# rgalljamov/DRLoco

Hardware: NVIDIA B200
Metric: env-steps/s incl. DeepMimic reward (higher is better)
Workload: dtype f32

## Files before the change

drloco_b200/csrc/fd_tree.cuh:

```cuda
#pragma once
#include "fd_common.cuh"

namespace drl {

template <int NV>
struct Topo;

template <>
struct Topo<14> {
  static constexpr int NB = 7, NCHAIN = 2, KMAX = 4, NROOT = 6, NSLIDE = 3;
  __host__ __device__ static constexpr int nd(int k) { return k == 0 ? 6 : (k == 1 ? 2 : 1); }
  __host__ __device__ static constexpr int dof_off(int k) { return k <= 1 ? 0 : (k == 2 ? 2 : (k == 3 ? 3 : 4)); }
  __host__ __device__ static constexpr int chain_dof0(int c) { return c == 0 ? 6 : 10; }
  __host__ __device__ static constexpr int chain_body1(int c) { return c == 0 ? 1 : 4; }
  __host__ __device__ static constexpr int chain_len(int) { return 4; }
  __host__ __device__ static constexpr int axis(int k, int s) { return k == 0 ? s : (k == 1 ? (s == 0 ? 1 : 0) : 1); }
  __host__ __device__ static constexpr int chain_of(int j) { return (j - 6) / 4; }
  static constexpr int NBOX = 2;
  __host__ __device__ static constexpr int box_body(int bx) { return bx == 0 ? 3 : 6; }
};

template <>
struct Topo<19> {
  static constexpr int NB = 8, NCHAIN = 3, KMAX = 4, NROOT = 6, NSLIDE = 3;
  __host__ __device__ static constexpr int nd(int k) { return k == 0 ? 6 : (k == 1 ? 3 : 1); }
  __host__ __device__ static constexpr int dof_off(int k) { return k <= 1 ? 0 : (k == 2 ? 3 : (k == 3 ? 4 : 5)); }
  __host__ __device__ static constexpr int chain_dof0(int c) { return c == 0 ? 9 : (c == 1 ? 14 : 6); }
  __host__ __device__ static constexpr int chain_body1(int c) { return c == 0 ? 2 : (c == 1 ? 5 : 1); }
  __host__ __device__ static constexpr int chain_len(int c) { return c == 2 ? 2 : 4; }
  __host__ __device__ static constexpr int axis(int k, int s) { return k == 0 ? s : (k == 1 ? (s == 2 ? 2 : -1) : 1); }
  __host__ __device__ static constexpr int chain_of(int j) { return j < 9 ? 2 : (j < 14 ? 0 : 1); }
  static constexpr int NBOX = 4;
  __host__ __device__ static constexpr int box_body(int bx) { return bx == 0 ? 0 : (bx == 1 ? 1 : (bx == 2 ? 4 : 7)); }
};

template <int NV>
__host__ __device__ constexpr unsigned body_subtree_mask(int b) {
  using T = Topo<NV>;
  if (b == 0) return (1u << T::NB) - 1u;
  unsigned m = 0;
  for (int c = 0; c < T::NCHAIN; c++)
    for (int k = 1; k < T::chain_len(c); k++) {
      const int x = T::chain_body1(c) + k - 1;
      if (x == b)
        for (int k2 = k; k2 < T::chain_len(c); k2++) m |= 1u << (T::chain_body1(c) + k2 - 1);
    }
  return m;
}

template <int NV>
__host__ __device__ constexpr bool dof_is_anc(int r, int k) {
  return r < k && (r < Topo<NV>::NROOT || Topo<NV>::chain_of(r) == Topo<NV>::chain_of(k));
}
template <int NV>
__host__ __device__ constexpr unsigned dof_anc_mask(int k) {
  unsigned m = 0;
  for (int r = 0; r < k; r++)
    if (dof_is_anc<NV>(r, k)) m |= 1u << r;
  return m;
}

template <int NV>
__host__ __device__ constexpr unsigned dof_desc_mask(int k) {
  unsigned m = 0;
  for (int c = k + 1; c < NV; c++)
    if (dof_is_anc<NV>(k, c)) m |= 1u << c;
  return m;
}

template <int NV, int G>
__device__ __forceinline__ float ldl_solve_tree(float (&H)[NV + 1], int l) {
  float invd = 0.f;
  const unsigned me = 1u << l;
#pragma unroll
  for (int k = NV - 1; k >= 0; k--) {
    const float dk = __shfl_sync(kFull, H[k], k, G);
    const float inv = fast_rcp(fmaxf(dk, 1e-30f));
    const float lck = H[k] * inv;
    const bool upd = (dof_anc_mask<NV>(k) & me) != 0u;
    if (l == k) invd = inv;
#pragma unroll
    for (int r = 0; r <= NV; r++) {
      if (r == NV || dof_is_anc<NV>(r, k)) {
        const float vr = __shfl_sync(kFull, H[r], k, G);
        if (upd) H[r] = fmaf(-vr, lck, H[r]);
      }
    }
  }
  float sacc = H[NV], x = 0.f;
#pragma unroll
  for (int k = 0; k < NV; k++) {
    const float xk = __shfl_sync(kFull, sacc * invd, k, G);
    if (dof_desc_mask<NV>(k) & me) sacc = fmaf(-H[k], xk, sacc);
    if (l == k) x = xk;
  }
  return x;
}

constexpr int kWredBox = 29;

template <int G>
struct EnvSmem {
  static constexpr int kWredHalf = (G == 16 ? 2 * kWredBox * 4 + 8 : 4 * kWredBox * 4);
  static_assert(kWredHalf % 32 == 16, "bank layout of the staging buffer");
  float v[G];
  float acc[G];
  float tau[G];
  float cssn[G][2];
  float S[G][12];
  union {
    struct {
      float Fd[G][12];
      float bodyR[kMaxBody][16];
      float Ib[kMaxBody][12];
      float axw[G][4];
    };
    struct {
      float Wred[2 * kWredHalf];
      float sph[G][12];
    };
  };
  float Ic[kMaxBody][12];
  union {
    struct {
      float V[kMaxBody][8];
      float Ab[kMaxBody][8];
      float T[kMaxBody][8];
      float W[kMaxBody][24];
      float U[kMaxBody][8];
    };
    float Mt[kMaxBody * 56];
  };
  float obsbuf[kMaxObs];
  int cnt[4];
  float pad_[(G == 16) ? 20 : 4];
};
static_assert((sizeof(EnvSmem<16>) / 4) % 32 == 8, "environment stride must be 8 mod 32 floats (bank layout)");
static_assert(sizeof(EnvSmem<16>) % 16 == 0 && sizeof(EnvSmem<32>) % 16 == 0, "vector loads need 16-byte rows");

struct ChainLane {
  int c3, row;
  int c6, comp;
};

__device__ __forceinline__ void rot_row(int ax, float& R0, float& R1, float& R2, float c, float s) {
  if (ax == 0) { const float u = R1, w = R2; R1 = c * u + s * w; R2 = c * w - s * u; }
  else if (ax == 1) { const float u = R2, w = R0; R2 = c * u + s * w; R0 = c * w - s * u; }
  else { const float u = R0, w = R1; R0 = c * u + s * w; R1 = c * w - s * u; }
}

template <int NV, int G>
__device__ __forceinline__ void tree_kinematics(const DevModel& M, EnvSmem<G>& E, const ChainLane& C, int l) {
  using T = Topo<NV>;
  if (l < 3 * T::NCHAIN) {
    const int c = C.c3, r = C.row;
    const int cd0 = T::chain_dof0(c), cb1 = T::chain_body1(c), clen = T::chain_len(c);
    float R0 = r == 0 ? 1.f : 0.f, R1 = r == 1 ? 1.f : 0.f, R2 = r == 2 ? 1.f : 0.f, pr = 0.f;
#pragma unroll
    for (int k = 0; k < T::KMAX; k++) {
      if (k < clen) {
        const int b = k == 0 ? 0 : cb1 + k - 1;
        const bool own = k > 0 || c == 0;
        if (k > 0) pr = pr + R0 * M.body_pos[b][0] + R1 * M.body_pos[b][1] + R2 * M.body_pos[b][2];
        const int j0 = k == 0 ? T::NSLIDE : cd0 + T::dof_off(k);
#pragma unroll
        for (int s = 0; s < 3; s++) {
          if (s < (k == 0 ? T::NROOT - T::NSLIDE : T::nd(k))) {
            const int j = j0 + s;
            const int code = M.dof_code[j];
            const float2 cs = *reinterpret_cast<const float2*>(&E.cssn[j][0]);
            const int a = T::axis(k, s) >= 0 ? T::axis(k, s) : (code & 3);
            const float ax = a == 0 ? R0 : (a == 1 ? R1 : R2);
            if (own) E.axw[j][r] = (code & 4) ? -ax : ax;
            rot_row(a, R0, R1, R2, cs.x, cs.y);
          }
        }
        if (own) *reinterpret_cast<float4*>(&E.bodyR[b][4 * r]) = make_float4(R0, R1, R2, pr);
      }
    }
  }
  __syncwarp();
}

template <int G>
__device__ __forceinline__ float body_point_z(const EnvSmem<G>& E, int b, const float* p) {
  const float4 r2 = *reinterpret_cast<const float4*>(&E.bodyR[b][8]);
  return r2.w + r2.x * p[0] + r2.y * p[1] + r2.z * p[2];
}

template <int NV, int G, bool PRE>
__device__ __forceinline__ void chain_prefix(EnvSmem<G>& E, const float* coef, float (*dst)[8], int c, int comp,
                                             float init) {
  using T = Topo<NV>;
  const int cd0 = T::chain_dof0(c), cb1 = T::chain_body1(c), clen = T::chain_len(c);
  float acc = init;
#pragma unroll
  for (int k = 0; k < T::KMAX; k++) {
    if (k < clen) {
      const int b = k == 0 ? 0 : cb1 + k - 1;
      const int j0 = k == 0 ? 0 : cd0 + T::dof_off(k);
      const bool own = k > 0 || c == 0;
#pragma unroll
      for (int s = 0; s < 6; s++) {
        if (s < T::nd(k)) {
          const int j = j0 + s;
          if (PRE && own) E.Fd[j][comp] = acc;
          acc = fmaf(coef[j], E.S[j][comp], acc);
        }
      }
      if (own) dst[b][comp] = acc;
    }
  }
}

template <int NV, int G>
__device__ __forceinline__ void chain_prefix_rows(EnvSmem<G>& E, float (*dst)[8], int c, int comp, float init) {
  using T = Topo<NV>;
  const int cd0 = T::chain_dof0(c), cb1 = T::chain_body1(c), clen = T::chain_len(c);
  float acc = init;
#pragma unroll
  for (int k = 0; k < T::KMAX; k++) {
    if (k < clen) {
      const int b = k == 0 ? 0 : cb1 + k - 1;
      const int j0 = k == 0 ? 0 : cd0 + T::dof_off(k);
#pragma unroll
      for (int s = 0; s < 6; s++)
        if (s < T::nd(k)) acc += E.Fd[j0 + s][comp];
      if (k > 0 || c == 0) dst[b][comp] = acc;
    }
  }
}

template <int NV>
__device__ __forceinline__ void subtree_scan(const float* src, float* dst, int stride, unsigned present) {
  using T = Topo<NV>;
  float root = (present & 1u) ? src[0] : 0.f;
#pragma unroll
  for (int c = 0; c < T::NCHAIN; c++) {
    float s = 0.f;
#pragma unroll
    for (int k = T::KMAX - 1; k >= 1; k--) {
      if (k < T::chain_len(c)) {
        const int b = T::chain_body1(c) + k - 1;
        if ((present >> b) & 1u) s += src[b * stride];
        dst[b * stride] = s;
      }
    }
    root += s;
  }
  dst[0] = root;
}

struct Contact {
  float Px, Py, Pz, D, mu, ar[4];
};
__device__ __forceinline__ void st_contact(float* p, const Contact& c) {
  *reinterpret_cast<float4*>(p) = make_float4(c.Px, c.Py, c.Pz, c.D);
  *reinterpret_cast<float4*>(p + 4) = make_float4(c.mu, c.ar[0], c.ar[1], c.ar[2]);
  p[8] = c.ar[3];
}
__device__ __forceinline__ Contact ld_contact(const float* p) {
  const float4 a = *reinterpret_cast<const float4*>(p), b = *reinterpret_cast<const float4*>(p + 4);
  return Contact{a.x, a.y, a.z, a.w, b.x, {b.y, b.z, b.w, p[8]}};
}

template <int G, bool BOX>
__device__ __forceinline__ void contact_setup(const DevModel& M, const EnvSmem<G>& E, int s, int b, float dist,
                                              Contact& c) {
  const float4 r0 = *reinterpret_cast<const float4*>(&E.bodyR[b][0]);
  const float4 r1 = *reinterpret_cast<const float4*>(&E.bodyR[b][4]);
  const float4 r2 = *reinterpret_cast<const float4*>(&E.bodyR[b][8]);
  const float x = M.cand_pos[s][0], y = M.cand_pos[s][1], z = M.cand_pos[s][2];
  if (BOX) {
    const float ux = M.cand_aux[s][0], uy = M.cand_aux[s][1], uz = M.cand_aux[s][2];
    c.Px = (r0.w + r0.x * ux + r0.y * uy + r0.z * uz) + (r0.x * x + r0.y * y + r0.z * z);
    c.Py = (r1.w + r1.x * ux + r1.y * uy + r1.z * uz) + (r1.x * x + r1.y * y + r1.z * z);
    c.Pz = (r2.w + r2.x * ux + r2.y * uy + r2.z * uz) + (r2.x * x + r2.y * y + r2.z * z) - 0.5f * dist;
  } else {
    const float rad = M.cand_aux[s][0];
    c.Px = r0.w + (r0.x * x + r0.y * y + r0.z * z);
    c.Py = r1.w + (r1.x * x + r1.y * y + r1.z * z);
    c.Pz = r2.w + (r2.x * x + r2.y * y + r2.z * z) - rad - 0.5f * dist;
  }
  const float mu = M.cand_mu[s];
  const float imp = impedance(M, dist);
  const float Rn = fmaxf(kMinVal, (1.f - imp) * M.body_invw_tran[b] * (1.f + mu * mu));
  c.D = imp * fast_rcp(2.f * mu * mu * Rn);
  c.mu = mu;
  const Vec6 Vb = ld6(E.V[b]);
  float ux, uy, uz;
  cross3(ux, uy, uz, Vb.w0, Vb.w1, Vb.w2, c.Px, c.Py, c.Pz);
// ... 204 lines not shown
  __syncwarp();
  float rhs0 = 0.f;
  if (L.isdof) {
    const float cb = dot6(S, ld6(E.Ab[L.body]));
    rhs0 = tau - M.dof_damping[l] * v - cb;
    if (DBG) { dbg[0 * 32 + l] = cb; dbg[1 * 32 + l] = rhs0; }
  }
  float lsg = 0.f, lD = 0.f, laref = 0.f;
  if (L.isdof && M.dof_limited[l]) {
    float dist = 0.f;
    const float lo = M.dof_lo[l], hi = M.dof_hi[l];
    if (q < lo) { lsg = 1.f; dist = q - lo; }
    else if (q > hi) { lsg = -1.f; dist = hi - q; }
    if (lsg != 0.f) {
      const float imp = impedance(M, dist);
      lD = imp * fast_rcp(fmaxf(kMinVal, (1.f - imp) * M.dof_invw[l]));
      laref = -M.Bc * lsg * v - M.Kc * imp * dist;
    }
  }
  if (!act0) AS.bits[0] = 0u;
  else if (!(AS.prev_act & 1u)) AS.bits[0] = 0xFu;
  if (!act1) AS.bits[1] = 0u;
  else if (!(AS.prev_act & 2u)) AS.bits[1] = 0xFu;
  if (lsg == 0.f) AS.lbit = false;
  else if (!AS.prev_lim) AS.lbit = true;
  const bool any_limit = __any_sync(kFull, lsg != 0.f);
  const bool constrained = (conmask != 0u) || any_limit;
  unsigned subcon = 0u;
#pragma unroll
  for (int b = 0; b < T::NB; b++)
    if (body_subtree_mask<NV>(b) & conmask) subcon |= 1u << b;
  int n_iter = 0;
  bool capped = false;
  if (solver_barrier) __syncthreads();
  float H[NV + 1];
  for (int it = 0; it < kMaxSolverIter; it++) {
    if (constrained) n_iter++;
    if (conmask != 0u) {
      float wv[28];
      contact_hessian(c0, act0 ? AS.bits[0] : 0u, wv);
      if (l < M.nbox_cand) {
        float* dst = &E.Wred[((l >> 2) & 1) * ES::kWredHalf + (l >> 3) * kWredBox * 4 + (l & 3)];
#pragma unroll
        for (int i = 0; i < 27; i++) dst[i * 4] = wv[i];
      }
      __syncwarp();
      if (!sph_any) {
#pragma unroll
        for (int i0 = 0; i0 < 27; i0 += G) {
          const int i = i0 + l;
          if (i < 27) {
            float sb[T::NBOX];
#pragma unroll
            for (int bx = 0; bx < T::NBOX; bx++) {
              const float4 x0 = *reinterpret_cast<const float4*>(&E.Wred[(bx * kWredBox + i) * 4]);
              const float4 x1 = *reinterpret_cast<const float4*>(&E.Wred[ES::kWredHalf + (bx * kWredBox + i) * 4]);
              sb[bx] = ((x0.x + x0.y) + (x0.z + x0.w)) + ((x1.x + x1.y) + (x1.z + x1.w));
            }
#pragma unroll
            for (int b = 0; b < T::NB; b++) {
              float tot = 0.f;
              bool any = false;
#pragma unroll
              for (int bx = 0; bx < T::NBOX; bx++)
                if ((body_subtree_mask<NV>(b) >> T::box_body(bx)) & 1u) { tot = any ? tot + sb[bx] : sb[bx]; any = true; }
              if (any) {
                if (i < 21) E.W[b][i] = tot; else E.U[b][i - 21] = tot;
              }
            }
          }
        }
        __syncwarp();
      } else {
        for (unsigned mk = conmask & ~M.box_body_mask; mk; mk &= mk - 1) {
          const int b = __ffs(mk) - 1;
          for (int i = l; i < 24; i += G) E.W[b][i] = 0.f;
          if (l < 8) E.U[b][l] = 0.f;
        }
#pragma unroll
        for (int bx = 0; bx < T::NBOX; bx++) {
#pragma unroll
          for (int i0 = 0; i0 < 27; i0 += G) {
            const int i = i0 + l;
            if (i < 27) {
              const float4 x0 = *reinterpret_cast<const float4*>(&E.Wred[(bx * kWredBox + i) * 4]);
              const float4 x1 = *reinterpret_cast<const float4*>(&E.Wred[ES::kWredHalf + (bx * kWredBox + i) * 4]);
              const float sum = ((x0.x + x0.y) + (x0.z + x0.w)) + ((x1.x + x1.y) + (x1.z + x1.w));
              const int b = T::box_body(bx);
              if (i < 21) E.W[b][i] = sum; else E.U[b][i - 21] = sum;
            }
          }
        }
        {
          float wv1[28];
          Contact c1 = {0.f, 0.f, 0.f, 0.f, 0.f, {0.f, 0.f, 0.f, 0.f}};
          const unsigned bt = act1 ? AS.bits[1] : 0u;
          if (bt) c1 = ld_contact(E.sph[l]);
          contact_hessian(c1, bt, wv1);
          const int b1 = M.cand_body[G + l < M.ncand ? G + l : 0];
          __syncwarp();
          for (unsigned sm = __ballot_sync(kFull, bt != 0u); sm; sm &= sm - 1) {
            if (wl == __ffs(sm) - 1) {
              float* Wb = E.W[b1];
              float* Ub = E.U[b1];
#pragma unroll
              for (int i = 0; i < 21; i++) Wb[i] += wv1[i];
#pragma unroll
              for (int i = 0; i < 6; i++) Ub[i] += wv1[21 + i];
            }
            __syncwarp();
          }
        }
        __syncwarp();
        const unsigned present = conmask | M.box_body_mask;
        for (int i = l; i < 27; i += G) {
          if (i < 21) subtree_scan<NV>(&E.W[0][i], &E.W[0][i], 24, present);
          else subtree_scan<NV>(&E.U[0][i - 21], &E.U[0][i - 21], 8, present);
        }
        __syncwarp();
      }
    }
    H[NV] = rhs0;
    if (L.isdof) {
      Vec6 F = inertia_mul(E.Ic[L.body], S);
      if ((subcon >> L.body) & 1u) {
        float Wl[24];
#pragma unroll
        for (int i = 0; i < 24; i += 4) {
          const float4 t = *reinterpret_cast<const float4*>(&E.W[L.body][i]);
          Wl[i] = t.x; Wl[i + 1] = t.y; Wl[i + 2] = t.z; Wl[i + 3] = t.w;
        }
        const float Sv[6] = {S.w0, S.w1, S.w2, S.v0, S.v1, S.v2};
        float y[6];
#pragma unroll
        for (int i = 0; i < 6; i++) {
          float t = 0.f;
#pragma unroll
          for (int j = 0; j < 6; j++) t = fmaf(Wl[sym6(i, j)], Sv[j], t);
          y[i] = t;
        }
        F.w0 += y[0]; F.w1 += y[1]; F.w2 += y[2]; F.v0 += y[3]; F.v1 += y[4]; F.v2 += y[5];
        H[NV] += dot6(S, ld6(E.U[L.body]));
      }
      st6(E.Fd[l], F);
    }
    __syncwarp();
    mass_column<NV, G>(M, E, L, S, H);
    if (AS.lbit) {
#pragma unroll
      for (int r = 0; r < NV; r++)
        if (r == l) H[r] += lD;
      H[NV] += lD * lsg * laref;
    }
    a = ldl_solve_tree<NV, G>(H, l);
    if (!L.isdof) a = 0.f;
    if (L.isdof) E.acc[l] = a;
    if (!constrained) break;
    __syncwarp();
    if (conmask != 0u) {
      if (iscomp) chain_prefix<NV, G, false>(E, E.acc, E.T, C.c6, C.comp, 0.f);
      __syncwarp();
    }
    bool changed = false;
    if (act0) {
      const unsigned nb = contact_rows(c0, ld6(E.T[body0]));
      changed = nb != AS.bits[0];
      AS.bits[0] = nb;
    }
    if (sph_any) {
      if (act1) {
        const Contact c1 = ld_contact(E.sph[l]);
        const unsigned nb = contact_rows(c1, ld6(E.T[M.cand_body[G + l]]));
        changed = changed || (nb != AS.bits[1]);
        AS.bits[1] = nb;
      }
    }
    {
      const bool nl = (lsg != 0.f) && (lsg * a - laref < 0.f);
      changed = changed || (nl != AS.lbit);
      AS.lbit = nl;
    }
    if (!__any_sync(kFull, changed)) break;
    if (it == kMaxSolverIter - 1 && env_any(changed, L.emask)) capped = true;
    __syncwarp();
  }
  AS.prev_act = (act0 ? 1u : 0u) | (act1 ? 2u : 0u);
  AS.prev_lim = lsg != 0.f;
  if (l == 0) { E.cnt[0] += n_iter; E.cnt[1] += capped ? 1 : 0; }
  if (DBG) {
    dbg[(2 + NV) * 32 + l] = a;
    if (l == 0) {
      dbg[(3 + NV) * 32 + 0] = zO;
      dbg[(3 + NV) * 32 + 1] = (float)__popc(conmask);
    }
    dbg[(4 + NV) * 32 + l] = (float)((act0 ? 1 : 0) + (act1 ? 1 : 0));
  }
}

template <int NV, int G>
__device__ __forceinline__ void pure_mass_column(const DevModel& M, EnvSmem<G>& E, const LaneConst& L,
                                                  const Vec6& S, float (&H)[NV + 1]) {
  __syncwarp();
  if (L.isdof) st6(E.Fd[L.l], inertia_mul(E.Ic[L.body], S));
  __syncwarp();
  mass_column<NV, G>(M, E, L, S, H);
  __syncwarp();
}

}
```

drloco_b200/csrc/mimic_step.cu:

```cuda
#include "fd_common.cuh"
#include "fd_tree.cuh"

namespace drl {

__device__ __forceinline__ unsigned long long mix64(unsigned long long x) {
  x += 0x9E3779B97F4A7C15ull;
  x = (x ^ (x >> 30)) * 0xBF58476D1CE4E5B9ull;
  x = (x ^ (x >> 27)) * 0x94D049BB133111EBull;
  return x ^ (x >> 31);
}

struct Cursor {
  int i_step, pos, count, ep_dur, rsi_step, n_det, resets, flags;
};

constexpr int kFlagReadStep0 = 4, kFlagDetEpisode = 8;
__device__ __forceinline__ int data_step(const Cursor& c) { return (c.flags & kFlagReadStep0) ? 0 : c.i_step; }
__device__ __forceinline__ int shift_step(const Cursor& c) { return (c.flags & kFlagDetEpisode) ? 0 : c.rsi_step; }

__device__ __forceinline__ void cursor_next(const DevModel& M, const StepArgs& A, Cursor& c, float& dist) {
  const int len = A.step_len[data_step(c)];
  c.pos += M.increment;
  if (M.cursor_mode == DRL_CURSOR_STEPWISE) {
    const int dif = c.pos - len + 1;
// ... 264 lines not shown
  float zO = M.root_z0;
  for (int j = 0; j < M.nslide; j++) zO = fmaf(M.dof_slide_z[j], E.cssn[j][1], zO);
  tree_kinematics<NV, G>(M, E, CL, l);
  float sz = 3.0e38f;
  for (int s = l; s < M.nsite; s += G) sz = fminf(sz, zO + body_point_z<G>(E, M.site_body[s], M.site_pos[s]));
  const float lowest = group_min<G>(sz);
  if (l == M.com_z_dof) q -= lowest;
  zoff = lowest;
  cursor_next(M, A, c, dist);
  __syncwarp();
}

#ifndef DRL_STEP_MAX_BLOCK
#define DRL_STEP_MAX_BLOCK 128
#endif
template <int NV, int G, bool RK4, bool DBG>
__global__ void __launch_bounds__(DRL_STEP_MAX_BLOCK, 512 / DRL_STEP_MAX_BLOCK) mimic_step_kernel(const StepArgs A, const int do_reset_only) {
  using ES = EnvSmem<G>;
  extern __shared__ __align__(16) unsigned char smem_raw[];
  DevModel& M = *reinterpret_cast<DevModel*>(smem_raw);
  constexpr int kModelBytes = (sizeof(DevModel) + 15) / 16 * 16;
  ES* envs = reinterpret_cast<ES*>(smem_raw + kModelBytes);
  {
    const int4* src = reinterpret_cast<const int4*>(A.model);
    int4* dst = reinterpret_cast<int4*>(smem_raw);
    for (int i = threadIdx.x; i < (int)(sizeof(DevModel) / 16); i += blockDim.x) dst[i] = src[i];
  }
  __syncthreads();
  const int epb = blockDim.x / G;
  const int eib = threadIdx.x / G;
  const int env_raw = blockIdx.x * epb + eib;
  const bool live = env_raw < A.num_envs;
  const int env = live ? env_raw : A.num_envs - 1;
  ES& E = envs[eib];
  LaneConst L;
  L.l = threadIdx.x % G;
  const int l = L.l;
  ChainLane CL;
  CL.c3 = l / 3; CL.row = l - 3 * CL.c3;
  CL.c6 = l / 6; CL.comp = l - 6 * CL.c6;
  L.emask = (G == 32) ? kFull : (0xFFFFu << (16 * ((threadIdx.x & 31) / 16)));
  L.isdof = l < M.nv;
  L.isbody = l < M.nb;
  const int jd = L.isdof ? l : 0;
  L.body = M.dof_body[jd]; L.type = M.dof_type[jd];

  float* sf = A.state_f + (size_t)env * (4 * G);
  int* si = A.state_i + (size_t)env * kCurCount8;
  float q = sf[l], v = sf[G + l], a = sf[2 * G + l];
  Cursor c;
  c.i_step = si[kCurIstep]; c.pos = si[kCurPos]; c.count = si[kCurCount]; c.ep_dur = si[kCurEpDur];
  c.rsi_step = si[kCurRsiStep]; c.n_det = si[kCurNDet]; c.resets = si[kCurResets]; c.flags = si[kCurFlags];
  float dist = sf[3 * G + kMiscDist], zoff = sf[3 * G + kMiscZoff];
  if (l == 0) { E.cnt[0] = 0; E.cnt[1] = 0; }
  int* sa = A.state_as + (size_t)env * G;
  ActiveSet AS;
  {
    const unsigned pk = (unsigned)sa[l];
    AS.bits[0] = pk & 0xFu; AS.bits[1] = (pk >> 4) & 0xFu; AS.prev_act = (pk >> 8) & 3u;
    AS.lbit = (pk >> 10) & 1u; AS.prev_lim = (pk >> 11) & 1u;
  }
  float* obs_out = A.obs + (size_t)env * M.obs_dim;

  if (do_reset_only) {
    const bool want = live && (A.reset_mask == nullptr || A.reset_mask[env]);
    if (!__any_sync(kFull, want)) return;
    reset_env<NV, G>(M, A, E, L, CL, env, c, q, v, dist, zoff);
    float ph, dv;
    build_obs<G>(M, A, E, L, c, q, v, ph, dv);
    const bool left = M.mirror_policy && A.left_step[c.i_step];
    write_obs<G>(M, E, l, left, want, obs_out);
    if (want) {
      sf[l] = q; sf[G + l] = v; sf[2 * G + l] = 0.f;
      if (l == 0) {
        sf[3 * G + kMiscDist] = dist; sf[3 * G + kMiscZoff] = zoff;
        sf[3 * G + kMiscWalked] = 0.f; sf[3 * G + kMiscEpRet] = 0.f; sf[3 * G + kMiscEpTor] = 0.f;
        sf[3 * G + kMiscPrevPos] = 1.f; sf[3 * G + kMiscPrevVel] = 1.f; sf[3 * G + kMiscPrevCom] = 1.f;
        if (A.ee_f) A.ee_f[2 * (size_t)env] = 1.f;
        si[kCurIstep] = c.i_step; si[kCurPos] = c.pos; si[kCurCount] = c.count; si[kCurEpDur] = 0;
        si[kCurRsiStep] = c.rsi_step; si[kCurNDet] = c.n_det; si[kCurResets] = c.resets; si[kCurFlags] = c.flags;
      }
    }
    return;
  }

  const bool left0 = M.mirror_policy && A.left_step[c.i_step];
  float force = 0.f;
  {
    float sc = 0.f;
    if (l < M.nu) {
      float act = A.actions[(size_t)env * M.act_dim + l];
      act = fminf(fmaxf(act, -1.f), 1.f);
      sc = act > 0.f ? __fmul_rn(act, M.act_chi[l]) : __fmul_rn(fabsf(act), M.act_clo[l]);
    }
    {
      const int src = l < M.nu ? M.mirror_act_idx[l] : 0;
      const float o = __shfl_sync(kFull, sc, src, G);
      if (left0) sc = l < M.nu ? M.mirror_act_sign[l] * o : 0.f;
    }
    E.tau[l] = 0.f;
    __syncwarp();
    if (l < M.nu) {
      const float cc = fminf(fmaxf(sc, M.act_clo[l]), M.act_chi[l]);
      force = fminf(fmaxf(M.act_gear[l] * cc, M.act_flo[l]), M.act_fhi[l]);
      E.tau[M.act_dof[l]] = M.act_gear[l] * force;
    }
    __syncwarp();
  }
  const float tau = E.tau[l];
  const float mean_abs_torque = group_sum<G>(l < M.nu ? fabsf(force) : 0.f) / (float)M.nu;

  const float h = M.timestep;
  bool bad = false;
  float* dbgp = (DBG && A.debug) ? A.debug + (size_t)env * 32 * 40 : nullptr;
  for (int sub = 0; sub < A.frame_skip; sub++) {
    {
      const bool blown = env_any(L.isdof && (!(fabsf(q) <= 1e10f) || !(fabsf(v) <= 1e10f)), L.emask);
      bad = bad || blown;
    }
    if (bad) { q = M.dof_ref[jd]; v = 0.f; a = 0.f; }
    if (RK4) {
      const float q0 = q, v0 = v;
      float accq = 0.f, accv = 0.f;
#pragma unroll 1
      for (int st = 0; st < 4; st++) {
        if (A.stage_barrier == 1) __syncthreads();
        Vec6 Sj;
        forward_dynamics<NV, G, DBG>(M, E, L, CL, q, v, tau, a, AS, Sj, dbgp, A.stage_barrier == 2);
        const float bw = (st == 0 || st == 3) ? (1.f / 6.f) : (1.f / 3.f);
        accq = fmaf(bw, v, accq);
        accv = fmaf(bw, a, accv);
        if (st < 3) {
          const float aw = st == 2 ? 1.f : 0.5f;
          const float vn = fmaf(h * aw, a, v0);
          q = fmaf(h * aw, v, q0);
          v = vn;
        }
      }
      q = fmaf(h, accq, q0);
      v = fmaf(h, accv, v0);
    } else {
      float Hc[NV + 1];
      float Ma = 0.f;
      Vec6 Sj;
      forward_dynamics<NV, G, DBG>(M, E, L, CL, q, v, tau, a, AS, Sj, dbgp, false);
      pure_mass_column<NV, G>(M, E, L, Sj, Hc);
#pragma unroll
      for (int r = 0; r < NV; r++) {
        if (DBG && dbgp) dbgp[(2 + r) * 32 + l] = Hc[r];
        Ma = fmaf(Hc[r], E.acc[r], Ma);
        if (r == l) Hc[r] += h * M.dof_damping[jd];
      }
      Hc[NV] = Ma;
      float an = ldl_solve_tree<NV, G>(Hc, l);
      if (!L.isdof) an = 0.f;
      v = fmaf(h, an, v);
      q = fmaf(h, v, q);
    }
  }
  {
    const bool blown = env_any(L.isdof && (!(fabsf(q) <= 1e10f) || !(fabsf(v) <= 1e10f)), L.emask);
    bad = bad || blown;
  }
  if (bad) { q = M.dof_ref[jd]; v = 0.f; a = 0.f; }

  float walked = sf[3 * G + kMiscWalked];
  float ep_ret = sf[3 * G + kMiscEpRet], ep_tor = sf[3 * G + kMiscEpTor];
  float pos_rew = sf[3 * G + kMiscPrevPos], vel_rew = sf[3 * G + kMiscPrevVel], com_rew = sf[3 * G + kMiscPrevCom];
  float reward, phase0 = 0.f, des0 = 0.f;
  float ov[2] = {0.f, 0.f};
  bool done;
  const int ep_dur_before = c.ep_dur;
  cursor_next(M, A, c, dist);
  if (ep_dur_before == 0) c.flags = (c.flags & 0xFFFF) | (c.pos << 16);
  if (A.playback) {
    float rq, rv;
    ref_lookup(M, A, c, dist, zoff, l, G, L.isdof, rq, rv);
    if (L.isdof) { q = rq; v = rv; }
  }
  build_obs<G>(M, A, E, L, c, q, v, phase0, des0);
  c.ep_dur += 1;
  {
    const float vx = __shfl_sync(kFull, v, 0, G), vy = __shfl_sync(kFull, v, 1, G);
    const float cx = fminf(fmaxf(vx, -5.5f), 5.5f), cy = fminf(fmaxf(vy, -5.5f), 5.5f);
    walked += sqrtf(cx * cx + cy * cy) * M.ctrl_freq_inv;
  }
  const float comz = __shfl_sync(kFull, q, M.com_z_dof, G);
  const bool timeout = c.ep_dur >= M.ep_dur_max;
  float rq, rv;
  ref_lookup(M, A, c, dist, zoff, l, G, L.isdof, rq, rv);
  bool et_low, et_trunk, et_drunk;
  {
    const int t0 = M.trunk_dof0;
    const float front_dev = fabsf(__shfl_sync(kFull, q - rq, t0, G));
    const float sag = __shfl_sync(kFull, q, t0 + 1, G), comy = __shfl_sync(kFull, q, 1, G);
    et_low = comz < 0.75f;
    et_trunk = (sag > 0.3f || sag < -0.05f) || front_dev > 0.2f;
    et_drunk = fabsf(comy) > 0.2f;
    if (A.playback) et_low = et_trunk = et_drunk = false;
  }
  const bool et_done = M.early_termination && (et_low || et_trunk || et_drunk);
  done = (comz < M.fall_z) || timeout || et_done;
  {
    const float dq = L.isdof ? q - rq : 0.f, dv = L.isdof ? v - rv : 0.f;
    const bool iscom = (M.com_mask >> l) & 1u;
    const float sp = group_sum<G>(iscom ? 0.f : dq * dq);
    const float sv = group_sum<G>(iscom ? 0.f : dv * dv);
    const float sc = group_sum<G>(iscom ? dq * dq : 0.f);
    if (!done && !bad) {
      pos_rew = expf(-3.f * sp);
      vel_rew = expf(-0.05f * sv);
      com_rew = expf(-16.f * sc);
    }
  }
  float ee_rew = 1.f;
  if (M.w_ee != 0.f) {
    ee_rew = A.ee_f[2 * (size_t)env];
    const float se = ee_sq_error<NV, G>(M, E, L, CL, q, rq);
    if (!done && !bad) ee_rew = expf(-M.ee_scale * se);
  }
  if (bad) {
    done = true;
    reward = 0.f;
  } else if (done) {
    reward = timeout ? 0.f : -0.f;
  } else {
    float imit = M.w_pos * pos_rew + M.w_vel * vel_rew + M.w_com * com_rew;
    if (M.w_ee != 0.f) imit = fmaf(M.w_ee, ee_rew, imit);
    reward = imit * M.rew_scale + M.alive_bonus;
  }
  {
    const bool left1 = M.mirror_policy && A.left_step[c.i_step];
    float* dst = (done && A.terminal_obs) ? A.terminal_obs + (size_t)env * M.obs_dim : obs_out;
    write_obs<G>(M, E, l, left1, live && !bad, dst, done ? nullptr : ov);
  }
  const int kRowStats = 2 * M.obs_dim + 2, kRowLen = kRowStats + DRL_STATS_COUNT;
  double* srow = reinterpret_cast<double*>(E.Mt);
  for (int i = l; i < kRowLen; i += G) srow[i] = 0.0;
  __syncwarp();
  ep_ret += reward;
  ep_tor += mean_abs_torque;
  const int ep_len_now = bad ? ep_dur_before + 1 : c.ep_dur;
  float med_tor = 0.f;
  if (A.tor_hist) {
    float* hist = A.tor_hist + (size_t)env * M.ep_dur_max;
    if (l == 0 && live && ep_dur_before < M.ep_dur_max) hist[ep_dur_before] = mean_abs_torque;
    __syncwarp();
    if (__any_sync(kFull, done)) {
      const int nh = ep_len_now < M.ep_dur_max ? ep_len_now : M.ep_dur_max;
      float* scratch = &E.S[0][0];
      const int cap = (int)((reinterpret_cast<float*>(E.Mt) - scratch)) - 256;
      med_tor = group_median<G>(hist, scratch, cap, (done && live) ? nh : 0, l);
    }
  }
  double* sd = A.state_d + (size_t)env * 4;
  if (l == 0 && live) {
    sd[0] += (double)pos_rew; sd[1] += (double)vel_rew; sd[2] += (double)com_rew; sd[3] += 1.0;
    if (A.ee_d) A.ee_d[env] += (double)ee_rew;
    srow[kRowStats + DRL_STAT_ENV_STEPS] = 1.0;
    srow[kRowStats + DRL_STAT_POS_REW_SUM] = (double)pos_rew;
    srow[kRowStats + DRL_STAT_VEL_REW_SUM] = (double)vel_rew;
    srow[kRowStats + DRL_STAT_COM_REW_SUM] = (double)com_rew;
    srow[kRowStats + DRL_STAT_REW_STEPS] = 1.0;
    srow[kRowStats + DRL_STAT_ABS_TORQUE_SUM] = (double)mean_abs_torque;
    srow[kRowStats + DRL_STAT_SOLVER_ITERS] = (double)E.cnt[0];
    srow[kRowStats + DRL_STAT_DYN_EVALS] = (double)(A.frame_skip * (RK4 ? 4 : 1));
    srow[kRowStats + DRL_STAT_SOLVER_CAPPED] = (double)E.cnt[1];
    if (!bad) {
      srow[kRowStats + DRL_STAT_ET_COM_LOW] = et_low ? 1.0 : 0.0;
      srow[kRowStats + DRL_STAT_ET_TRUNK] = et_trunk ? 1.0 : 0.0;
      srow[kRowStats + DRL_STAT_ET_DRUNK] = et_drunk ? 1.0 : 0.0;
    }
    if (A.vn_ret) {
      const float r = A.vn_ret[env] * A.vn_gamma + reward;
      A.vn_ret[env] = done ? 0.f : r;
      srow[2 * M.obs_dim] = (double)r;
      srow[2 * M.obs_dim + 1] = (double)r * (double)r;
    }
    if (A.extras) {
      float* ex = A.extras + (size_t)env * 16;
      ex[0] = pos_rew; ex[1] = vel_rew; ex[2] = com_rew; ex[3] = walked; ex[4] = mean_abs_torque;
      ex[5] = des0; ex[6] = phase0; ex[7] = zoff;
    }
  }
  if (done && l == 0 && live) {
    const int ep_len = ep_len_now;
    float* ms = sf + 3 * G;
    const int fl = c.flags;
    auto smooth = [&](int slot, int bit, float nv, float f) {
      ms[slot] = (fl >> bit) & 1 ? f * nv + (1.f - f) * ms[slot] : nv;
    };
    if (ep_len > 1) { smooth(kMiscMeanRewSm, 0, ep_ret / (float)(ep_len - 1), 0.9f); c.flags |= 1; }
    smooth(kMiscPosSm, 1, (float)(sd[0] / sd[3]), 0.9f);
    smooth(kMiscVelSm, 1, (float)(sd[1] / sd[3]), 0.9f);
    smooth(kMiscComSm, 1, (float)(sd[2] / sd[3]), 0.9f);
    smooth(kMiscEpRetSm, 1, ep_ret, 0.25f);
    smooth(kMiscEpLenSm, 1, (float)ep_len, 0.75f);
    smooth(kMiscTorSm, 1, ep_tor / (float)ep_len, 0.75f);
    if (A.tor_hist) A.med_tor_sm[env] = (fl >> 1) & 1 ? 0.75f * med_tor + 0.25f * A.med_tor_sm[env] : med_tor;
    if (A.ee_f) {
      const float nv = (float)(A.ee_d[env] / sd[3]);
      float& sm = A.ee_f[2 * (size_t)env + 1];
      sm = (fl >> 1) & 1 ? 0.9f * nv + (1.f - 0.9f) * sm : nv;
    }
    c.flags |= 2;
    ms[kMiscMoved] = walked;
    srow[kRowStats + DRL_STAT_EPISODES] = 1.0;
// ... 259 lines not shown
```

Measured before the change: 17.37 million.

## Restructure tree LDL solve to eliminate chains in parallel and solve root block per lane

Replaces the serial per-dof LDL factorization, which shuffles a column at every one of NV steps, with a scheme that exploits the branch structure. All chains are eliminated in lockstep over the maximum chain length. The reduced root rows are then staged through shared scratch (E.Mt), and every lane solves the small 6x6 root block redundantly in registers. The goal is fewer sequential shuffle rounds and a shorter dependency chain, at the cost of extra register arrays, shared-memory traffic, warp syncs and reuse of the Mt union region as scratch.

```diff
diff --git a/drloco_b200/csrc/fd_tree.cuh b/drloco_b200/csrc/fd_tree.cuh
--- a/drloco_b200/csrc/fd_tree.cuh
+++ b/drloco_b200/csrc/fd_tree.cuh
@@ -61,40 +61,157 @@
 }
 
 template <int NV>
-__host__ __device__ constexpr unsigned dof_desc_mask(int k) {
-  unsigned m = 0;
-  for (int c = k + 1; c < NV; c++)
-    if (dof_is_anc<NV>(k, c)) m |= 1u << c;
-  return m;
+__host__ __device__ constexpr int chain_nd(int c) { return Topo<NV>::dof_off(Topo<NV>::chain_len(c)); }
+template <int NV>
+__host__ __device__ constexpr int chain_nd_max() {
+  int n = 0;
+  for (int c = 0; c < Topo<NV>::NCHAIN; c++) n = chain_nd<NV>(c) > n ? chain_nd<NV>(c) : n;
+  return n;
+}
+template <int NV>
+__host__ __device__ constexpr bool chains_same_nd() {
+  for (int c = 1; c < Topo<NV>::NCHAIN; c++)
+    if (chain_nd<NV>(c) != chain_nd<NV>(0)) return false;
+  return true;
+}
+
+template <int NV>
+__host__ __device__ constexpr int last_chain() {
+  int p = 0;
+  for (int c = 1; c < Topo<NV>::NCHAIN; c++)
+    if (Topo<NV>::chain_dof0(c) > Topo<NV>::chain_dof0(p)) p = c;
+  return p;
 }
 
 template <int NV, int G>
-__device__ __forceinline__ float ldl_solve_tree(float (&H)[NV + 1], int l) {
+__device__ __forceinline__ float ldl_solve_tree(float (&H)[NV + 1], int l, float* scratch) {
+  using T = Topo<NV>;
+  constexpr int NR = T::NROOT, NC = T::NCHAIN, ND = chain_nd_max<NV>(), P = last_chain<NV>();
+  static_assert(T::chain_dof0(P) + chain_nd<NV>(P) == NV, "the last chain holds the highest dofs");
+  static_assert(NR + 2 <= 8 && 8 * G <= kMaxBody * 56, "scratch rows: 8 floats per lane");
+  const bool chainl = l >= NR && l < NV;
+  const bool rootl = l < NR;
+  const int cown = chainl ? T::chain_of(l) : P;
+  const int f0 = T::chain_dof0(cown);
+  const int nown = chains_same_nd<NV>() ? chain_nd<NV>(P) : chain_nd<NV>(cown);
+  const int pos = chainl ? l - f0 : (rootl ? -1 : ND);
+  float R[NR], C[NC][ND], z = H[NV];
+#pragma unroll
+  for (int r = 0; r < NR; r++) R[r] = H[r];
+#pragma unroll
+  for (int c = 0; c < NC; c++)
+#pragma unroll
+    for (int j = 0; j < ND; j++) C[c][j] = j < chain_nd<NV>(c) ? H[T::chain_dof0(c) + j] : 0.f;
+#pragma unroll
+  for (int c = 0; c < NC; c++)
+    if (c != P) {
+#pragma unroll
+      for (int j = 0; j < ND; j++) C[P][j] = cown == c ? C[c][j] : C[P][j];
+    }
+
   float invd = 0.f;
-  const unsigned me = 1u << l;
-#pragma unroll
-  for (int k = NV - 1; k >= 0; k--) {
-    const float dk = __shfl_sync(kFull, H[k], k, G);
-    const float inv = fast_rcp(fmaxf(dk, 1e-30f));
-    const float lck = H[k] * inv;
-    const bool upd = (dof_anc_mask<NV>(k) & me) != 0u;
-    if (l == k) invd = inv;
-#pragma unroll
-    for (int r = 0; r <= NV; r++) {
-      if (r == NV || dof_is_anc<NV>(r, k)) {
-        const float vr = __shfl_sync(kFull, H[r], k, G);
-        if (upd) H[r] = fmaf(-vr, lck, H[r]);
+#pragma unroll
+  for (int m = 0; m < ND; m++) {
+    const int pown = nown - 1 - m;
+    float hk = 0.f;
+#pragma unroll
+    for (int j = 0; j < ND; j++)
+      if (j == pown) hk = C[P][j];
+    const float invl = fast_rcp(fmaxf(hk, 1e-30f));
+    if (pos == pown) invd = invl;
+    const bool upd = pos < pown;
+    const int src = f0 + pown;
+    const float lck = hk * __shfl_sync(kFull, invl, src, G);
+#pragma unroll
+    for (int r = 0; r < NR; r++) {
+      const float v = __shfl_sync(kFull, R[r], src, G);
+      if (upd) R[r] = fmaf(-v, lck, R[r]);
+    }
+    {
+      const float v = __shfl_sync(kFull, z, src, G);
+      if (upd) z = fmaf(-v, lck, z);
+    }
+#pragma unroll
+    for (int j = 0; j < ND - 1 - m; j++) {
+      const float v = __shfl_sync(kFull, C[P][j], src, G);
+      if (upd && j < pown) C[P][j] = fmaf(-v, lck, C[P][j]);
+    }
+#pragma unroll
+    for (int c = 0; c < NC; c++) {
+      if (c != P && m < chain_nd<NV>(c)) {
+        const int pc = chain_nd<NV>(c) - 1 - m, srcc = T::chain_dof0(c) + pc;
+        const float lckc = C[c][pc] * __shfl_sync(kFull, invl, srcc, G);
+#pragma unroll
+        for (int j = 0; j < pc; j++) {
+          const float v = __shfl_sync(kFull, C[P][j], srcc, G);
+          C[c][j] = rootl ? fmaf(-v, lckc, C[c][j]) : C[c][j];
+        }
       }
     }
   }
-  float sacc = H[NV], x = 0.f;
-#pragma unroll
-  for (int k = 0; k < NV; k++) {
-    const float xk = __shfl_sync(kFull, sacc * invd, k, G);
-    if (dof_desc_mask<NV>(k) & me) sacc = fmaf(-H[k], xk, sacc);
-    if (l == k) x = xk;
-  }
-  return x;
+
+  __syncwarp();
+  float4* row = reinterpret_cast<float4*>(scratch + 8 * l);
+  row[0] = make_float4(R[0], R[1], R[2], R[3]);
+  row[1] = make_float4(R[4], R[5], z, invd);
+  __syncwarp();
+#pragma unroll
+  for (int k = T::chain_dof0(P) - 1; k >= NR; k--) {
+    const int c = T::chain_of(k), j = k - T::chain_dof0(c);
+    const float4 a = *reinterpret_cast<const float4*>(scratch + 8 * k);
+    const float4 b = *reinterpret_cast<const float4*>(scratch + 8 * k + 4);
+    const float lck = C[c][j] * b.w;
+    const float v[NR + 1] = {a.x, a.y, a.z, a.w, b.x, b.y, b.z};
+#pragma unroll
+    for (int r = 0; r < NR; r++) R[r] = rootl ? fmaf(-v[r], lck, R[r]) : R[r];
+    z = rootl ? fmaf(-v[NR], lck, z) : z;
+  }
+  __syncwarp();
+
+  row[0] = make_float4(R[0], R[1], R[2], R[3]);
+  row[1] = make_float4(R[4], R[5], z, invd);
+  __syncwarp();
+  float A[NR][8];
+#pragma unroll
+  for (int s = 0; s < NR; s++) {
+    const float4 a = *reinterpret_cast<const float4*>(scratch + 8 * s);
+    const float4 b = *reinterpret_cast<const float4*>(scratch + 8 * s + 4);
+    A[s][0] = a.x; A[s][1] = a.y; A[s][2] = a.z; A[s][3] = a.w; A[s][4] = b.x; A[s][5] = b.y; A[s][6] = b.z;
+  }
+  float ir[NR];
+#pragma unroll
+  for (int k = NR - 1; k >= 0; k--) {
+    ir[k] = fast_rcp(fmaxf(A[k][k], 1e-30f));
+#pragma unroll
+    for (int s = 0; s < k; s++) {
+      const float lck = A[s][k] * ir[k];
+#pragma unroll
+      for (int r = 0; r < k; r++) A[s][r] = fmaf(-A[k][r], lck, A[s][r]);
+      A[s][NR] = fmaf(-A[k][NR], lck, A[s][NR]);
+    }
+  }
+  float xr[NR], xme = 0.f;
+#pragma unroll
+  for (int k = 0; k < NR; k++) {
+    float t = A[k][NR];
+#pragma unroll
+    for (int r = 0; r < k; r++) t = fmaf(-A[k][r], xr[r], t);
+    xr[k] = t * ir[k];
+    if (l == k) xme = xr[k];
+  }
+
+  const float4 ra = row[0], rb = row[1];
+  const float rr[NR] = {ra.x, ra.y, ra.z, ra.w, rb.x, rb.y};
+  float sacc = rb.z;
+  invd = rb.w;
+#pragma unroll
+  for (int r = 0; r < NR; r++) sacc = fmaf(-rr[r], xr[r], sacc);
+#pragma unroll
+  for (int d = 0; d < ND - 1; d++) {
+    const float xd = __shfl_sync(kFull, sacc * invd, f0 + d, G);
+    if (pos > d) sacc = fmaf(-C[P][d], xd, sacc);
+  }
+  return rootl ? xme : sacc * invd;
 }
 
 constexpr int kWredBox = 29;
@@ -137,6 +254,8 @@
 };
 static_assert((sizeof(EnvSmem<16>) / 4) % 32 == 8, "environment stride must be 8 mod 32 floats (bank layout)");
 static_assert(sizeof(EnvSmem<16>) % 16 == 0 && sizeof(EnvSmem<32>) % 16 == 0, "vector loads need 16-byte rows");
+static_assert(offsetof(EnvSmem<16>, Mt) % 16 == 0 && offsetof(EnvSmem<32>, Mt) % 16 == 0,
+              "ldl_solve_tree reads its root block from E.Mt with 16-byte loads");
 
 struct ChainLane {
   int c3, row;
@@ -647,7 +766,7 @@
         if (r == l) H[r] += lD;
       H[NV] += lD * lsg * laref;
     }
-    a = ldl_solve_tree<NV, G>(H, l);
+    a = ldl_solve_tree<NV, G>(H, l, E.Mt);
     if (!L.isdof) a = 0.f;
     if (L.isdof) E.acc[l] = a;
     if (!constrained) break;
diff --git a/drloco_b200/csrc/mimic_step.cu b/drloco_b200/csrc/mimic_step.cu
--- a/drloco_b200/csrc/mimic_step.cu
+++ b/drloco_b200/csrc/mimic_step.cu
@@ -440,7 +440,7 @@
         if (r == l) Hc[r] += h * M.dof_damping[jd];
       }
       Hc[NV] = Ma;
-      float an = ldl_solve_tree<NV, G>(Hc, l);
+      float an = ldl_solve_tree<NV, G>(Hc, l, E.Mt);
       if (!L.isdof) an = 0.f;
       v = fmaf(h, an, v);
       q = fmaf(h, v, q);
```

Measured after the change: 17.41 million (median of 6 runs). About the same (+0.3%).
